# locuslab/mpc.pytorch

Measured on AMD Instinct MI355X. Metric: LQR problem-steps/sec (batch*T/s), n_state=12 n_ctrl=4 T=50, higher is better.
Workload: dtype f32

## Files before the change

### mpc.pytorch_amd/csrc/capi.hip

```cpp
#include <algorithm>
#include <atomic>
#include <cmath>
#include <cstdio>
#include <cstdlib>
#include <cstring>
#include <string>

#include "lqr_common.h"

namespace mpclqr {
static thread_local std::string g_last_error;
void set_last_error(const char *msg) { g_last_error = msg ? msg : ""; }

static int fail(int code, const char *msg)
{
    set_last_error(msg);
    return code;
}

template <typename F>
static int by_dtype(int dtype, F &&f)
{
    return dtype == MPC_F32 ? f(float()) : f(double());
}

struct EnvSwitch { const char *name; char a, b; int unset; };
static const EnvSwitch SW_DPP16_RING = {"MPC_DPP16_RING", '2', '4', 0};
static const EnvSwitch SW_MFMA40_RING = {"MPC_MFMA40_RING", '2', '3', 0};
static const EnvSwitch SW_DPP16_RESIDENT = {"MPC_DPP16_RESIDENT", '0', '1', -1};
static int read_switch(const EnvSwitch &s)
{
    const char *e = getenv(s.name);
    return (e && (e[0] == s.a || e[0] == s.b)) ? e[0] - '0' : s.unset;
}

struct DeviceFacts {
    int ring_force;
    int simds;
    int ring40_force;
    bool sticky;
    int resident;
};
static const DeviceFacts &device_facts()
{
    static DeviceFacts f = [] {
        DeviceFacts d;
        d.simds = 1024;
        hipDeviceProp_t prop;
        int dev = 0;
        if (hipGetDevice(&dev) == hipSuccess && hipGetDeviceProperties(&prop, dev) == hipSuccess && prop.multiProcessorCount > 0)
            d.simds = prop.multiProcessorCount * 4;
        d.ring_force = read_switch(SW_DPP16_RING);
        d.ring40_force = read_switch(SW_MFMA40_RING);
        d.sticky = getenv("MPC_DPP16_RING_DYNAMIC") == nullptr;
        d.resident = read_switch(SW_DPP16_RESIDENT);
        return d;
    }();
    return f;
}
static int env_switch(const EnvSwitch &s, int at_load) { return device_facts().sticky ? at_load : read_switch(s); }

#ifndef MPC_DPP16_RESIDENT_DEFAULT
#define MPC_DPP16_RESIDENT_DEFAULT 1
#endif
static std::atomic<int64_t> g_resident_launches{0};
static bool dpp16_resident(const StepParams<float> &q)
{
    const DeviceFacts &f = device_facts();
    int on = env_switch(SW_DPP16_RESIDENT, f.resident);
    const int waves = (q.B + 3) / 4;
    if (on < 0) on = (MPC_DPP16_RESIDENT_DEFAULT && 16 * (long)waves > 15 * (long)f.simds) ? 1 : 0;
    return on != 0 && q.bound_mode == MPC_BOUND_NONE && !q.zero_mask && q.T >= 2 && q.T <= 64  && !q.sweep_only &&
           (q.B + 3) / 4 <= f.simds;
}

static int mfma40_ring(const StepParams<float> &sp)
{
    const DeviceFacts &f = device_facts();
    const int force = env_switch(SW_MFMA40_RING, f.ring40_force);
    if (force) return force;
    if (sp.bound_mode != MPC_BOUND_NONE) return sp.B > f.simds ? 2 : 3;
    return (sp.B > f.simds && sp.B <= f.simds + f.simds / 2) ? 2 : 3;
}

static int check_problem(const mpc_lqr_problem *p, bool need_cost, bool need_nominal, bool need_F = true)
{
    if (!p) return fail(MPC_E_NULL, "problem is NULL");
    if (p->B < 0 || p->T < 1 || p->ns < 1 || p->nc < 1) return fail(MPC_E_DIMS, "need B>=0, T>=1, ns>=1, nc>=1");
    if (p->nc > 64) return fail(MPC_E_DIMS, "n_ctrl > 64 is not supported");
    if (p->dtype != MPC_F32 && p->dtype != MPC_F64) return fail(MPC_E_DTYPE, "dtype must be MPC_F32 or MPC_F64");
    if (p->B == 0) return MPC_OK;
    if (need_cost && (!p->C || !p->c)) return fail(MPC_E_NULL, "C / c is NULL");
    if (need_F && p->T > 1 && !p->F) return fail(MPC_E_NULL, "F is NULL");
    if (!p->x_init) return fail(MPC_E_NULL, "x_init is NULL");
    if (need_nominal && (!p->cur_x || !p->cur_u)) return fail(MPC_E_NULL, "current_x / current_u is NULL");
    return MPC_OK;
}

static int check_env(const mpc_env_dynamics *e, int ns, int nc)
{
    const int kind = e->kind & ~MPC_ENV_CTRL_CARRY, carry = (e->kind & MPC_ENV_CTRL_CARRY) ? 1 : 0;
    if (kind < MPC_ENV_PENDULUM || kind > MPC_ENV_CARTPOLE) return fail(MPC_E_ARG, "unknown simulator kind");
    if (!e->params) return fail(MPC_E_NULL, "simulator params is NULL");
    if (nc != 1 || ns != env_ns(kind) + carry) return fail(MPC_E_DIMS, "n_state / n_ctrl do not match the simulator");
    if (!(e->dt > 0) || !(e->u_max >= 0)) return fail(MPC_E_ARG, "simulator dt / u_max");
    return MPC_OK;
}

static int check_env_points(const mpc_env_dynamics *env, int dtype, int64_t N)
{
    if (!env) return fail(MPC_E_NULL, "simulator is NULL");
    if (dtype != MPC_F32 && dtype != MPC_F64) return fail(MPC_E_DTYPE, "bad dtype");
    if (env->kind & MPC_ENV_CTRL_CARRY) return fail(MPC_E_UNSUPPORTED, "MPC_ENV_CTRL_CARRY: linearise the simulator itself (the carry block is constant)");
    if (env->kind < MPC_ENV_PENDULUM || env->kind > MPC_ENV_CARTPOLE) return fail(MPC_E_ARG, "unknown simulator kind");
    const int rc = check_env(env, env_ns(env->kind), 1);
    if (rc) return rc;
    return N < 0 ? fail(MPC_E_DIMS, "N < 0") : MPC_OK;
}

static int check_options(const mpc_lqr_problem *p, const mpc_lqr_options *o)
{
    if (!o) return MPC_OK;
    if (o->bound_mode < MPC_BOUND_NONE || o->bound_mode > MPC_BOUND_TENSOR) return fail(MPC_E_ARG, "bad bound_mode");
    if (o->bound_mode == MPC_BOUND_TENSOR && (!o->lo || !o->hi) && p->B > 0) return fail(MPC_E_NULL, "tensor bounds are NULL");
    if (o->max_linesearch_iter < 1) return fail(MPC_E_ARG, "max_linesearch_iter must be > 0");
    if (o->delta_u == o->delta_u && o->delta_u >= 0 && o->bound_mode == MPC_BOUND_NONE)
        return fail(MPC_E_ARG, "delta_u requires u_lower/u_upper (mpc/lqr_step.py:195)");
    if (o->true_dynamics) {
        int rc = check_env(o->true_dynamics, p->ns, p->nc);
        if (rc) return rc;
    }
    return MPC_OK;
}


static mpc_lqr_problem sizes_only(int B, int T, int ns, int nc, int dtype)
{
    mpc_lqr_problem q;
    memset(&q, 0, sizeof(q));
    q.B = B; q.T = T; q.ns = ns; q.nc = nc; q.dtype = dtype;
    return q;
}
template <typename real>
static StepParams<real> sizes_only(const StepParams<real> &sp)
{
    const mpc_lqr_problem q = sizes_only(sp.B, sp.T, sp.ns, sp.nc, sizeof(real) == 4 ? MPC_F32 : MPC_F64);
    StepParams<real> s = make_params<real>(&q, nullptr, nullptr);
    s.env.kind = sp.env.kind;
    return s;
}

struct WsLayout { int64_t K, k, Kk, bytes, qp, qp_st, qp_sb; };
static WsLayout layout_generic(int64_t TB, int B, int ns, int nc, int64_t e) { return {0, TB * nc * ns * e, -1, TB * nc * (ns + 1) * e, -1, 0, 0}; }
static WsLayout layout_row(int64_t TB, int B, int ns, int nc, int64_t e) { return {0, TB * nc * ns * e, 0, TB * nc * (ns + 1) * e * 9, -1, 0, 0}; }
static WsLayout layout_fused12(int64_t TB, int B, int ns, int nc, int64_t e) { return {0, TB * nc * ns * e, 0, e == 4 ? TB * (128 + 16) * 4 : TB * 64 * 8, -1, 0, 0}; }
static WsLayout layout_dpp16(int64_t TB, int B, int ns, int nc, int64_t e) { return {0, TB * nc * ns * e, 0, layout_fused12(TB, B, ns, nc, e).bytes, 48 * 4, (int64_t)B * 64, 64}; }
static WsLayout layout_mfma40(int64_t TB, int B, int ns, int nc, int64_t e)
{
    const WsLayout w = layout_generic(TB, B, ns, nc, e);
    return {w.K, w.k, w.bytes, w.bytes + TB * (328 + 40) * 4, w.k, (int64_t)B * nc, nc};
}
static WsLayout layout_pad40(int64_t TB, int B, int ns, int nc, int64_t e)
{
    const int64_t k = TB * 256 * 4, Kk = k + TB * 8 * 4;
    return {0, k, Kk, Kk + TB * (328 + 40) * 4, k, (int64_t)B * 8, 8};
}

static bool row_kernel_pays(long lds_bytes, int B)
{
    const long per_cu = (160L * 1024) / lds_bytes;
    return (B + 3) / 4 <= (device_facts().simds / 4) * (per_cu < 8 ? per_cu : 8);
}
static bool wave1_pays(const StepParams<float> &sp) { return wave1_supported(sp) && row_kernel_pays(wave1_lds_bytes(sp), sp.B); }
static bool wave1_pays(const StepParams<double> &) { return false; }
static bool wave1_carry_pays(const StepParams<float> &sp) { return wave1_carry_supported(sp) && row_kernel_pays(wave1_carry_lds_bytes(sp), sp.B); }

static int dpp16_ring(const StepParams<float> &sp)
{
    const bool constrained = sp.bound_mode != MPC_BOUND_NONE || sp.zero_mask != nullptr;
    const int force = env_switch(SW_DPP16_RING, device_facts().ring_force);
    return (force ? force == 2 : (!constrained || (sp.B + 3) / 4 > device_facts().simds)) ? 2 : 4;
}
static int launch_dpp16(const StepRoute &r, const StepParams<float> &q, hipStream_t st)
{
    if (r.ring == 2 && dpp16_resident(q)) {
        g_resident_launches.fetch_add(1, std::memory_order_relaxed);
        return launch_step_dpp16_res(q, st);
    }
    return r.ring == 2 ? launch_step_dpp16_ring2(q, st) : launch_step_dpp16(q, st);
}

enum StepFamily { FAM_NONE, FAM_GENERIC, FAM_ROW , FAM_FUSED12 ,
                  FAM_MFMA40 , FAM_PAD40  };
enum {
    K_SIMULATOR = 1,
    K_CARRIES = 2,
    K_CARRY_ONLY = 4,
    K_SWEEP_STOP = 8,
    K_PARKS_STATUS = 16,
    K_SIZES_QUERY = 32,
    K_SIZES_RECORD = 64,
};
struct StepRefusal { int code; const char *text; };
template <typename real>
struct StepKernelIn {
    bool (*rule)(const StepParams<real> &);
    int (*launch)(const StepRoute &, const StepParams<real> &, hipStream_t);
    bool needs_workspace;
// ... 772 lines not shown
                       const void *gf, void *gparams, void *workspace, int64_t workspace_bytes, void *stream)
{
    const int rc = check_env_points(env, dtype, N);
    if (rc || N == 0) return rc;
    if (!x || !u || !gF || !gf || !gparams || !workspace) return fail(MPC_E_NULL, "env_param_grad: NULL argument");
    if (workspace_bytes < env_param_grad_workspace_bytes(N))
        return fail(MPC_E_DIMS, "workspace too small (see mpc_env_param_grad_workspace_bytes)");
    if ((uintptr_t)workspace % 8) return fail(MPC_E_ARG, "env_param_grad: the workspace must be 8-byte aligned");
    return by_dtype(dtype, [&](auto t) {
        typedef decltype(t) real;
        EnvDesc<real> e;
        set_env(e, env);
        return launch_env_param_grad<real>(e, (long)N, (const real *)x, (const real *)u, (const real *)gF, (const real *)gf, (real *)gparams,
                                           (double *)workspace, (hipStream_t)stream);
    });
}

int64_t mpc_mlp_workspace_bytes(const mpc_mlp_dynamics *net) { return nn_workspace_bytes(net); }

int mpc_mlp_supported(const mpc_mlp_dynamics *net, int n_state, int n_ctrl) { return nn_budget(net, n_state, n_ctrl); }

int mpc_mlp_rollout(const mpc_lqr_problem *p, const mpc_lqr_options *o, const mpc_mlp_dynamics *net, const void *K,
                    const void *k, const void *old_costs, const mpc_lqr_outputs *out, void *workspace,
                    int64_t workspace_bytes, void *stream)
{
    if (!p || !out) return fail(MPC_E_NULL, "problem / outputs is NULL");
    if (p->B < 0 || p->T < 1 || p->ns < 1 || p->nc < 1) return fail(MPC_E_DIMS, "need B>=0, T>=1, ns>=1, nc>=1");
    if (p->dtype != MPC_F32) return fail(MPC_E_DTYPE, "the network kernels are fp32 only");
    if (p->B == 0) return MPC_OK;
    if (!p->x_init || !p->cur_u) return fail(MPC_E_NULL, "x_init / current_u is NULL");
    if ((p->C == nullptr) != (p->c == nullptr)) return fail(MPC_E_NULL, "pass both C and c, or neither");
    if (!out->new_x) return fail(MPC_E_NULL, "new_x is NULL");
    if ((K == nullptr) != (k == nullptr)) return fail(MPC_E_NULL, both_gains);
    if (K) {
        if (!p->cur_x || !p->C || !old_costs || !out->new_u)
            return fail(MPC_E_NULL, "line search needs current_x, C, c, old_costs and new_u");
        int rc = check_options(p, o);
        if (rc) return rc;
        if (o && o->true_dynamics) return fail(MPC_E_ARG, "mpc_mlp_rollout: options.true_dynamics must be NULL");
    }
    StepParams<float> sp = make_params<float>(p, K ? o : nullptr, out);
    sp.K = (float *)K;
    sp.k = (float *)k;
    sp.old_costs_in = (const float *)old_costs;
    return launch_nn_rollout(sp, net, workspace, workspace_bytes, (hipStream_t)stream);
}

int mpc_mlp_linearize(const mpc_mlp_dynamics *net, int n_state, int n_ctrl, int64_t N, const void *x, const void *u,
                      void *F, void *f, void *workspace, int64_t workspace_bytes, void *stream)
{
    if (n_state < 1 || n_ctrl < 1 || N < 0) return fail(MPC_E_DIMS, "need n_state>=1, n_ctrl>=1, N>=0");
    if (N == 0) return MPC_OK;
    if (!x || !u || !F || !f) return fail(MPC_E_NULL, "mlp_linearize: NULL argument");
    return launch_nn_linearize(net, (long)N, n_state, n_ctrl, (const float *)x, (const float *)u, (float *)F, (float *)f,
                               workspace, workspace_bytes, (hipStream_t)stream);
}

int mpc_mlp_linearize_carry(const mpc_mlp_dynamics *net, int n_state, int n_ctrl, int64_t N, const void *z, const void *u,
                            void *aF, void *af, void *workspace, int64_t workspace_bytes, void *stream)
{
    if (n_state < 1 || n_ctrl < 1 || N < 0) return fail(MPC_E_DIMS, "need n_state>=1, n_ctrl>=1, N>=0");
    if (n_state + n_ctrl > 32) return fail(MPC_E_DIMS, "mlp_linearize_carry: n_state + n_ctrl <= 32 (the augmented state of the step kernels)");
    if (N == 0) return MPC_OK;
    if (!z || !u || !aF || !af) return fail(MPC_E_NULL, "mlp_linearize_carry: NULL argument");
    return launch_nn_linearize_carry(net, (long)N, n_state, n_ctrl, (const float *)z, (const float *)u, (float *)aF, (float *)af,
                                     workspace, workspace_bytes, (hipStream_t)stream);
}

int64_t mpc_mlp_param_grad_workspace_bytes(const mpc_mlp_dynamics *net, int64_t N) { return nn_param_grad_workspace_bytes(net, N); }

int mpc_mlp_param_grad(const mpc_mlp_dynamics *net, int n_state, int n_ctrl, int64_t N, const void *x, const void *u,
                       const void *gF, const void *gf, const mpc_mlp_param_grads *out, void *workspace,
                       int64_t workspace_bytes, void *stream)
{
    if (n_state < 1 || n_ctrl < 1 || N < 0) return fail(MPC_E_DIMS, "need n_state>=1, n_ctrl>=1, N>=0");
    if (!net || !out || !workspace) return fail(MPC_E_NULL, "mlp_param_grad: NULL argument");
    if (N > 0 && (!x || !u || !gF || !gf)) return fail(MPC_E_NULL, "mlp_param_grad: NULL argument");
    if (net->n_layers >= 1 && net->n_layers <= MPC_MLP_MAX_LAYERS)
        for (int l = 0; l < net->n_layers; ++l)
            if (!out->gW[l] || !out->gb[l]) return fail(MPC_E_NULL, "mlp_param_grad: gradient pointer is NULL");
    return launch_nn_param_grad(net, (long)N, n_state, n_ctrl, (const float *)x, (const float *)u, (const float *)gF,
                                (const float *)gf, out, workspace, workspace_bytes, (hipStream_t)stream);
}

int mpc_lqr_kkt_prepare(int dtype, int B, int T, int ns, int nc, const void *dl_dx, const void *dl_du,
                        const void *u_star, const mpc_lqr_options *o, void *negr, uint8_t *mask, void *stream)
{
    if (dtype != MPC_F32 && dtype != MPC_F64) return fail(MPC_E_DTYPE, "bad dtype");
    if (B < 0 || T < 1 || ns < 1 || nc < 1) return fail(MPC_E_DIMS, "bad dims");
    if (B == 0) return MPC_OK;
    if (!dl_dx || !dl_du || !negr) return fail(MPC_E_NULL, "kkt_prepare: NULL argument");
    const int mode = o ? o->bound_mode : MPC_BOUND_NONE;
    if (mask && (mode == MPC_BOUND_NONE || !u_star)) return fail(MPC_E_ARG, "kkt_prepare: mask needs bounds and u*");
    if (mask && mode == MPC_BOUND_TENSOR && (!o->lo || !o->hi)) return fail(MPC_E_NULL, "tensor bounds are NULL");
    return by_dtype(dtype, [&](auto t) {
        typedef decltype(t) real;
        return launch_kkt_prepare<real>(B, T, ns, nc, (const real *)dl_dx, (const real *)dl_du, (const real *)u_star, mode, o ? (real)o->lo_s : 0,
                                        o ? (real)o->hi_s : 0, o ? (const real *)o->lo : nullptr, o ? (const real *)o->hi : nullptr, (real *)negr,
                                        mask, (hipStream_t)stream);
    });
}

int mpc_pnqp_lu(int dtype, int B, int n, const void *H, const void *q, const void *lo, const void *hi,
                const void *x0, int n_iter, void *x, uint8_t *If_out, int32_t *iters, int32_t *status,
                void *Hfree, void *LU, int32_t *pivots, void *stream)
{
    if (dtype != MPC_F32 && dtype != MPC_F64) return fail(MPC_E_DTYPE, "bad dtype");
    if (B < 0 || n < 1) return fail(MPC_E_DIMS, "bad dims");
    if (B == 0) return MPC_OK;
    if (!H || !q || !lo || !hi || !x) return fail(MPC_E_NULL, "pnqp: NULL argument");
    if (n_iter < 1) n_iter = 20;
    return by_dtype(dtype, [&](auto t) {
        typedef decltype(t) real;
        return launch_pnqp<real>(B, n, (const real *)H, (const real *)q, (const real *)lo, (const real *)hi, (const real *)x0, n_iter, (real *)x,
                                 If_out, iters, status, (real *)Hfree, (real *)LU, pivots, (hipStream_t)stream);
    });
}

int mpc_pnqp(int dtype, int B, int n, const void *H, const void *q, const void *lo, const void *hi,
             const void *x0, int n_iter, void *x, uint8_t *If_out, int32_t *iters, int32_t *status,
             void *Hfree, void *stream)
{
    return mpc_pnqp_lu(dtype, B, n, H, q, lo, hi, x0, n_iter, x, If_out, iters, status, Hfree, nullptr, nullptr, stream);
}

int mpc_traj_cost(const mpc_lqr_problem *p, void *x, void *cost, void *stream)
{
    if (!p) return fail(MPC_E_NULL, "problem is NULL");
    int rc = check_problem(p, cost != nullptr, false);
    if (rc) return rc;
    if (p->B == 0) return MPC_OK;
    if (!p->cur_u) return fail(MPC_E_NULL, "traj_cost: u (cur_u) is NULL");
    hipStream_t st = (hipStream_t)stream;
    if (p->dtype == MPC_F32) {
        StepParams<float> sp = make_params<float>(p, nullptr, nullptr);
        if (!cost && x && traj_wave_supported(sp)) return launch_traj_wave(sp, (float *)x, st);
        return launch_traj_cost<float>(sp, (float *)x, (float *)cost, st);
    }
    StepParams<double> sp = make_params<double>(p, nullptr, nullptr);
    return launch_traj_cost<double>(sp, (double *)x, (double *)cost, st);
}

int mpc_select_best(int dtype, int B, int T, int ns, int nc, int first, double best_cost_eps, const void *x,
                    const void *u, const void *costs, const void *du_norm, void *best_x, void *best_u,
                    void *best_costs, void *best_du_norm, void *flags, void *host_flags, int32_t host_tag,
                    const int32_t *status, void *stream)
{
    if (dtype != MPC_F32 && dtype != MPC_F64) return fail(MPC_E_DTYPE, "bad dtype");
    if (B < 0 || T < 1 || ns < 1 || nc < 1) return fail(MPC_E_DIMS, "bad dims");
    if (B == 0) return MPC_OK;
    if (!x || !u || !costs || !du_norm || !best_x || !best_u || !best_costs || !best_du_norm || !flags)
        return fail(MPC_E_NULL, "select_best: NULL argument");
    if ((uintptr_t)flags & 7 || (uintptr_t)host_flags & 7) return fail(MPC_E_ARG, "select_best: the flags blocks must be 8-byte aligned");
    return by_dtype(dtype, [&](auto t) {
        typedef decltype(t) real;
        return launch_select_best<real>(B, T, ns, nc, first, (real)best_cost_eps, (const real *)x, (const real *)u, (const real *)costs,
                                        (const real *)du_norm, (real *)best_x, (real *)best_u, (real *)best_costs, (real *)best_du_norm, flags,
                                        host_flags, host_tag, status, (hipStream_t)stream);
    });
}

int mpc_du_norm_reference(int dtype, int T, int B, int nc, const void *u, const void *new_u, void *out, void *stream)
{
    if (dtype != MPC_F32 && dtype != MPC_F64) return fail(MPC_E_DTYPE, "bad dtype");
    if (B < 0 || T < 1 || nc < 1) return fail(MPC_E_DIMS, "bad dims");
    if (B == 0) return MPC_OK;
    if (!u || !new_u || !out) return fail(MPC_E_NULL, "du_norm_reference: NULL argument");
    hipStream_t st = (hipStream_t)stream;
    if (dtype == MPC_F32) return launch_du_norm_reference<float>(T, B, nc, (const float *)u, (const float *)new_u, (float *)out, st);
    return launch_du_norm_reference<double>(T, B, nc, (const double *)u, (const double *)new_u, (double *)out, st);
}

}
```

### mpc.pytorch_amd/csrc/lqr_common.h

```cpp
#pragma once
#include <hip/hip_runtime.h>
#include <stdint.h>
#include "../../include/mpc_lqr.h"
#include "lqr_params.h"

namespace mpclqr {

void set_last_error(const char *msg);

enum { MPC_IMPL_AUTO = 0, MPC_IMPL_GENERIC = 1, MPC_IMPL_MFMA16 = 2, MPC_IMPL_DPP16 = 3, MPC_IMPL_TINY = 4, MPC_IMPL_MFMA40 = 5,
       MPC_IMPL_WAVE1 = 6, MPC_IMPL_MFMA40_PAD = 7, MPC_IMPL_DPP16_PAD = 8,
       MPC_IMPL_MFMA40_NARROW = 9,
       MPC_IMPL_WAVE1_CARRY = 10 };

struct StepRoute {
    int code; const char *msg;
    int kernel;
    int phase;
    int ring;
    bool pad16;
    bool needs_resolve;
    int64_t K_off, k_off;
    int64_t Kk_off, status_off;
    int64_t qp_off, qp_st, qp_sb;
};
template <typename real>
StepRoute step_route(const StepParams<real> &sp, const mpc_lqr_problem *p, int impl, int phase_mask, const void *workspace,
                     int64_t workspace_bytes);

struct KktPointers {
    const void *dl_dx, *dl_du, *dC, *dc, *dF, *df, *dx_init, *dx_out, *du_out, *workspace;
};
struct KktRoute {
    int code; const char *msg;
    bool no_kernel;
    int kernel;
    int64_t bytes;
};
KktRoute kkt_fused_route(const StepParams<float> &sp, const mpc_lqr_problem *p, const KktPointers &a, int64_t workspace_bytes);
KktRoute kkt_fused_route_kernel(const StepParams<float> &sp, const mpc_lqr_problem *p, const KktPointers &a, int64_t workspace_bytes,
                                int kernel);

template <typename real> int launch_step_generic(const StepParams<real> &p, int phase_mask, hipStream_t st);
template <typename real> int launch_pnqp(int B, int n, const real *H, const real *q, const real *lo,
                                         const real *hi, const real *x0, int n_iter, real *x,
                                         uint8_t *If_out, int *iters, int *status, real *Hfree,
                                         real *LU, int *pivots, hipStream_t st);
template <typename real> int launch_traj_cost(const StepParams<real> &p, real *x, real *cost, hipStream_t st);
template <typename real> int launch_kkt_grads(const StepParams<real> &p, const real *dx, const real *du,
                                              const real *dl_dx, const real *dl_du, real *dC, real *dc,
                                              real *dF, real *df, real *dx_init, hipStream_t st);
template <typename real> int launch_kkt_prepare(int B, int T, int ns, int nc, const real *dl_dx,
                                                const real *dl_du, const real *u_star, int bound_mode,
                                                real lo_s, real hi_s, const real *lo, const real *hi,
                                                real *negr, uint8_t *mask, hipStream_t st);
template <typename real> int launch_select_best(int B, int T, int ns, int nc, int first, real eps,
                                                const real *x, const real *u, const real *costs,
                                                const real *du_norm, real *bx, real *bu, real *bc,
                                                real *bd, void *flags, void *host_flags, int host_tag, const int *status,
                                                hipStream_t st);
template <typename real> int launch_du_norm_reference(int T, int B, int nc, const real *u, const real *new_u, real *out, hipStream_t st);
template <typename real> int launch_env_linearize(const EnvDesc<real> &env, long N, const real *x, const real *u,
                                                  real *F, real *f, hipStream_t st);
int64_t env_param_grad_workspace_bytes(int64_t N);
template <typename real> int launch_env_param_grad(const EnvDesc<real> &env, long N, const real *x, const real *u,
                                                   const real *gF, const real *gf, real *gparams, double *ws, hipStream_t st);
size_t generic_lds_bytes(int ns, int nc, size_t elem);
template <typename real> int launch_slew_augment(const mpc_lqr_problem *p, double gamma, real *aC, real *ac, real *aF, real *af, hipStream_t st);

bool dpp16_supported(const StepParams<float> &p);
int launch_step_dpp16(const StepParams<float> &p, hipStream_t st);
int launch_step_dpp16_ring2(const StepParams<float> &p, hipStream_t st);
bool dpp16_pad_supported(const StepParams<float> &p);
int launch_step_dpp16_res(const StepParams<float> &p, hipStream_t st);
int launch_step_dpp16_pad(const StepParams<float> &p, hipStream_t st);
bool kkt_dpp16_supported(const StepParams<float> &p, const float *dx, const float *du, const float *dl_dx,
                         const float *dC, const float *dF);
int launch_kkt_dpp16(const StepParams<float> &p, const float *dx, const float *du, const float *dl_dx, float *dC,
                     float *dc, float *dF, float *df, float *dx_init, hipStream_t st);

bool kkt_fused_dpp16_supported(const StepParams<float> &p, const float *dl_dx, const float *dl_du, const float *dC,
                               const float *dF, const float *ws);
int64_t kkt_fused_dpp16_workspace_bytes(int T, int B);
bool kkt_fused_dpp16_pad_supported(const StepParams<float> &p, const float *ws);
int launch_kkt_fused_dpp16_pad(const StepParams<float> &p, const float *dl_dx, const float *dl_du, float *dC, float *dc, float *dF,
                               float *df, float *dx_init, float *dx_out, float *du_out, float *ws, float decay, int max_ls,
                               hipStream_t st);
int launch_kkt_fused_dpp16(const StepParams<float> &p, const float *dl_dx, const float *dl_du, float *dC, float *dc, float *dF,
                           float *df, float *dx_init, float *dx_out, float *du_out, float *ws, float decay, int max_ls,
                           hipStream_t st);

bool tiny_supported(int ns, int nc);
template <typename real> int launch_step_tiny(const StepParams<real> &p, hipStream_t st);
bool wave1_supported(const StepParams<float> &p);
long wave1_lds_bytes(const StepParams<float> &p);
int launch_step_wave1(const StepParams<float> &p, hipStream_t st);
bool wave1_carry_supported(const StepParams<float> &p);
long wave1_carry_lds_bytes(const StepParams<float> &p);
int launch_step_wave1_carry(const StepParams<float> &p, hipStream_t st);

bool traj_wave_supported(const StepParams<float> &p);
int launch_traj_wave(const StepParams<float> &p, float *x, hipStream_t st);
bool kkt_wave_supported(const StepParams<float> &p, const float *dx, const float *du, const float *dl_dx, const float *dC,
                        const float *dF);
int launch_kkt_wave(const StepParams<float> &p, const float *dx, const float *du, const float *dl_dx, float *dC,
                    float *dc, float *dF, float *df, float *dx_init, hipStream_t st);

int launch_kkt_costates(const StepParams<float> &p, const float *dx, const float *du, const float *dl_dx, float *park, float *dx_init,
                        hipStream_t st);
int kkt_shared_partials(int T, int B);
int64_t kkt_shared_workspace_bytes(int T, int B, int ns, int nc);
int launch_kkt_shared(const StepParams<float> &p, const float *dx, const float *du, const float *dl_dx, float *sum_dC, float *sum_dc,
                      float *sum_dF, float *sum_df, float *dx_init, void *workspace, hipStream_t st);

int launch_kkt_outer(const StepParams<float> &p, const float *dx, const float *du, float *dC, float *dc, float *dF, hipStream_t st);

bool mfma40_supported(const StepParams<float> &p);
int launch_step_mfma40(const StepParams<float> &p, hipStream_t st);
int launch_step_mfma40_ring2(const StepParams<float> &p, hipStream_t st);
bool mfma40_pad_supported(const StepParams<float> &p);
bool mfma40_pad16_supported(const StepParams<float> &p);
int launch_step_mfma40_pad4(const StepParams<float> &p, hipStream_t st);
int launch_step_mfma40_pad16(const StepParams<float> &p, hipStream_t st);
bool mfma40_narrow_supported(const StepParams<float> &p);
int launch_step_mfma40_narrow4(const StepParams<float> &p, hipStream_t st);
int launch_step_mfma40_narrow16(const StepParams<float> &p, hipStream_t st);
bool kkt_fused_mfma40_supported(const StepParams<float> &p, const float *dl_dx, const float *dl_du, const float *dC,
                                const float *dF, const float *ws);
int64_t kkt_fused_mfma40_workspace_bytes(int T, int B);
bool kkt_fused_mfma40_pad_supported(const StepParams<float> &p, const float *ws);
bool kkt_fused_mfma40_pad16_supported(const StepParams<float> &p, const float *ws);
int launch_kkt_fused_mfma40_pad16(const StepParams<float> &p, const float *dl_dx, const float *dl_du, float *dC, float *dc, float *dF,
                                  float *df, float *dx_init, float *dx_out, float *du_out, float *ws, float decay, int max_ls,
                                  hipStream_t st);
int launch_kkt_fused_mfma40_pad(const StepParams<float> &p, const float *dl_dx, const float *dl_du, float *dC, float *dc, float *dF,
                                float *df, float *dx_init, float *dx_out, float *du_out, float *ws, float decay, int max_ls,
                                hipStream_t st);
int launch_kkt_fused_mfma40(const StepParams<float> &p, const float *dl_dx, const float *dl_du, float *dC, float *dc, float *dF,
                            float *df, float *dx_init, float *dx_out, float *du_out, float *ws, float decay, int max_ls,
                            hipStream_t st);
bool kkt_fused_mfma40_narrow_supported(const StepParams<float> &p, const float *ws);
bool kkt_fused_mfma40_narrow16_supported(const StepParams<float> &p, const float *ws);
int64_t kkt_fused_mfma40_narrow_workspace_bytes(int T, int B);
int launch_kkt_fused_mfma40_narrow16(const StepParams<float> &p, const float *dl_dx, const float *dl_du, float *dC, float *dc, float *dF,
                                     float *df, float *dx_init, float *dx_out, float *du_out, float *ws, float decay, int max_ls,
                                     hipStream_t st);
int launch_kkt_fused_mfma40_narrow4(const StepParams<float> &p, const float *dl_dx, const float *dl_du, float *dC, float *dc, float *dF,
                                    float *df, float *dx_init, float *dx_out, float *du_out, float *ws, float decay, int max_ls,
                                    hipStream_t st);

int nn_budget(const mpc_mlp_dynamics *net, int ns, int nc);
int64_t nn_workspace_bytes(const mpc_mlp_dynamics *net);
int launch_nn_rollout(const StepParams<float> &p, const mpc_mlp_dynamics *net, void *workspace, int64_t bytes, hipStream_t st);
int launch_nn_linearize(const mpc_mlp_dynamics *net, long N, int ns, int nc, const float *x, const float *u, float *F,
                        float *f, void *workspace, int64_t bytes, hipStream_t st);
int launch_nn_linearize_carry(const mpc_mlp_dynamics *net, long N, int ns, int nc, const float *z, const float *u, float *aF,
                              float *af, void *workspace, int64_t bytes, hipStream_t st);
int64_t nn_param_grad_workspace_bytes(const mpc_mlp_dynamics *net, int64_t N);
int launch_nn_param_grad(const mpc_mlp_dynamics *net, long N, int ns, int nc, const float *x, const float *u, const float *gF,
                         const float *gf, const mpc_mlp_param_grads *out, void *workspace, int64_t bytes, hipStream_t st);

bool mfma16_supported(const StepParams<float> &p);
int launch_step_mfma16(const StepParams<float> &p, hipStream_t st);
bool mfma16_supported(const StepParams<double> &p);
int launch_step_mfma16(const StepParams<double> &p, hipStream_t st);

}
```

### mpc.pytorch_amd/csrc/lqr_generic.hip

```cpp
#include "lqr_common.h"

namespace mpclqr {

namespace {

constexpr int WAVE = 64;
constexpr int MAX_THREADS = 256;

inline int threads_for(int ns, int nc) { return (ns + nc) > 24 ? MAX_THREADS : WAVE; }

template <typename real> __device__ __forceinline__ real rabs(real x) { return x < 0 ? -x : x; }
template <typename real> __device__ __forceinline__ real rsqrt_(real x);
template <> __device__ __forceinline__ float rsqrt_<float>(float x) { return sqrtf(x); }
template <> __device__ __forceinline__ double rsqrt_<double>(double x) { return sqrt(x); }

template <typename real> __device__ __forceinline__ real eclamp(real x, real lo, real hi)
{
    if (x < lo) x = lo;
    if (x > hi) x = hi;
    return x;
}

typedef float mfma_acc_t __attribute__((ext_vector_type(4)));
template <class LA, class LB>
// ... 699 lines not shown
    const int ir = i < ns ? i : 0;
    const bool hasf = p.f != nullptr;
    const bool isu = i >= ns && i < n;
    const real *aux0 = isu ? p.cur_u + (long)b * nc + (i - ns) : (hasf && i < ns ? p.f + (long)b * p.f_sb + i : p.x_init);
    const long aux_st = isu ? (long)B * nc : (hasf && i < ns ? p.f_st : 0);
    const bool auxv = isu || (hasf && i < ns);
    const real *F0 = p.F + (long)b * p.F_sb + (long)ir * n;
    auto load_stage = [&](int t, int slot) {
        t = t < T - 2 ? t : T - 2;
        const real *Ft = F0 + (long)t * p.F_st;
        if constexpr (VEC) {
            const float4 *F4 = reinterpret_cast<const float4 *>(Ft);
#pragma unroll
            for (int q = 0; q < 4; ++q) {
                const float4 v = F4[q];
                row[slot][4 * q] = v.x, row[slot][4 * q + 1] = v.y, row[slot][4 * q + 2] = v.z, row[slot][4 * q + 3] = v.w;
            }
        } else {
#pragma unroll
            for (int j = 0; j < 16; ++j) row[slot][j] = Ft[j < n ? j : 0];
        }
        aux[slot] = aux0[(long)t * aux_st];
    };
    auto advance = [&](int t, int slot) {
        const real a = auxv ? aux[slot] : (real)0;
        const real tau = i < ns ? xi : a;
        real acc = i < ns ? a : (real)0;
#pragma unroll
        for (int j = 0; j < 16; ++j) acc += (VEC || j < n ? row[slot][j] : (real)0) * __shfl(tau, j, 16);
        xi = acc;
        if (own) x[((long)(t + 1) * B + b) * ns + i] = xi;
    };
#pragma unroll
    for (int d = 0; d < DEPTH; ++d) load_stage(d, d);
    int t0 = 0;
    for (; t0 + DEPTH <= T - 1; t0 += DEPTH) {
#pragma unroll
        for (int d = 0; d < DEPTH; ++d) {
            advance(t0 + d, d);
            load_stage(t0 + d + DEPTH, d);
        }
    }
#pragma unroll
    for (int d = 0; d < DEPTH - 1; ++d)
        if (t0 + d < T - 1) advance(t0 + d, d);
}

template <typename real>
__global__ void __launch_bounds__(MAX_THREADS)
kkt_grads_kernel(StepParams<real> p, const real *dx, const real *du, const real *dl_dx, const real *dl_du,
                 real *dC, real *dc, real *dF, real *df, real *dx_init)
{
    extern __shared__ __attribute__((aligned(16))) char smem_raw[];
    Smem<real> s;
    s.carve(smem_raw, p.ns, p.nc, blockDim.x);
    const int b = blockIdx.x, tid = threadIdx.x, nt = blockDim.x;
    const int ns = p.ns, nc = p.nc, n = ns + nc, T = p.T, B = p.B;
    if (b >= B) return;
    real *lam = s.xn, *dlam = s.dxv, *lam2 = s.xn2, *dlam2 = s.v;
    bool have = false;
    for (int t = T - 1; t >= 0; --t) {
        const long tb = (long)t * B + b;
        const real *Ct = p.C + (long)t * p.C_st + (long)b * p.C_sb;
        const real *ct = p.c + (long)t * p.c_st + (long)b * p.c_sb;
        for (int e = tid; e < n * n; e += nt) s.Q[e] = Ct[e];
        if (have) {
            const real *Ft = p.F + (long)t * p.F_st + (long)b * p.F_sb;
            for (int e = tid; e < ns * n; e += nt) s.F[e] = Ft[e];
        }
        for (int i = tid; i < n; i += nt) {
            s.tau[i] = i < ns ? p.cur_x[tb * ns + i] : p.cur_u[tb * nc + (i - ns)];
            s.dtau[i] = i < ns ? dx[tb * ns + i] : du[tb * nc + (i - ns)];
        }
        __syncthreads();
        for (int e = tid; e < n * n; e += nt) {
            const int i = e / n, j = e - i * n;
            dC[tb * n * n + e] = (real)-0.5 * (s.dtau[i] * s.tau[j] + s.tau[i] * s.dtau[j]);
        }
        for (int i = tid; i < n; i += nt) dc[tb * n + i] = -s.dtau[i];
        for (int i = tid; i < ns; i += nt) {
            real r1 = 0, r2 = 0;
            for (int j = 0; j < n; ++j) {
                r1 += s.Q[i * n + j] * s.tau[j];
                r2 += s.Q[i * n + j] * s.dtau[j];
            }
            r1 += ct[i];
            r2 -= dl_dx[tb * ns + i];
            if (have)
                for (int m = 0; m < ns; ++m) {
                    r1 += s.F[m * n + i] * lam[m];
                    r2 += s.F[m * n + i] * dlam[m];
                }
            lam2[i] = r1;
            dlam2[i] = r2;
        }
        if (have) {
            for (int e = tid; e < ns * n; e += nt) {
                const int i = e / n, j = e - i * n;
                dF[tb * ns * n + e] = -(dlam[i] * s.tau[j] + lam[i] * s.dtau[j]);
            }
            if (df)
                for (int i = tid; i < ns; i += nt) df[tb * ns + i] = -dlam[i];
        }
        __syncthreads();
        for (int i = tid; i < ns; i += nt) { lam[i] = lam2[i]; dlam[i] = dlam2[i]; }
        __syncthreads();
        have = true;
    }
    for (int i = tid; i < ns; i += nt) dx_init[(long)b * ns + i] = -dlam[i];
}

template <typename real>
__global__ void kkt_prepare_kernel(long TB, int ns, int nc, const real *dl_dx, const real *dl_du,
                                   const real *u_star, int bound_mode, real lo_s, real hi_s,
                                   const real *lo, const real *hi, real *negr, uint8_t *mask)
{
    const int n = ns + nc;
    const long total = TB * n;
    for (long e = (long)blockIdx.x * blockDim.x + threadIdx.x; e < total; e += (long)gridDim.x * blockDim.x) {
        const long tb = e / n;
        const int i = (int)(e - tb * n);
        if (i < ns) {
            negr[e] = -dl_dx[tb * ns + i];
        } else {
            const long ui = tb * nc + (i - ns);
            negr[e] = -dl_du[ui];
            if (mask) {
                const real l = bound_mode == MPC_BOUND_SCALAR ? lo_s : lo[ui];
                const real h = bound_mode == MPC_BOUND_SCALAR ? hi_s : hi[ui];
                const real u = u_star[ui];
                mask[ui] = (rabs<real>(u - l) <= (real)1e-8 || rabs<real>(u - h) <= (real)1e-8) ? 1 : 0;
            }
        }
    }
}

template <typename real> struct BitsOf;
template <> struct BitsOf<float> { using type = unsigned int; };
template <> struct BitsOf<double> { using type = unsigned long long; };

constexpr int kSelPB = 8;

template <typename real> struct SelectArgs {
    int B, T, ns, nc, first;
    real eps;
    const real *x, *u, *costs, *du;
    real *bx, *bu, *bc, *bd;
    const int *status;
    unsigned char *flags, *host;
    int host_tag;
};

template <typename real, typename vec>
__global__ void __launch_bounds__(256) select_best_kernel(SelectArgs<real> a, int owners_only)
{
    constexpr int VW = sizeof(vec) / sizeof(real);
    const int tid = threadIdx.x;
    if (blockIdx.x == 0 && !owners_only) {
        __shared__ real s_max[4];
        __shared__ int s_fl[4];
        const volatile real *bc = a.bc;
        real d = 0;
        int fl = 0;
        for (int b = tid; b < a.B; b += 256) {
            real v = a.du[b];
            if (a.first || a.costs[b] <= bc[b] + a.eps) fl |= 1;
            if (v != v) { fl |= 2; v = 0; }
            d = v > d ? v : d;
            if (a.status && (a.status[b] & (MPC_ST_C_ASYMMETRIC | MPC_ST_C_TESTED)) != MPC_ST_C_TESTED) fl |= 4;
        }
        for (int off = 32; off > 0; off >>= 1) {
            const real o = __shfl_down(d, off);
            d = o > d ? o : d;
            fl |= __shfl_down(fl, off);
        }
        if ((tid & 63) == 0) s_max[tid >> 6] = d, s_fl[tid >> 6] = fl;
        __syncthreads();
        if (tid == 0) {
            for (int w = 1; w < 4; ++w) d = s_max[w] > d ? s_max[w] : d, fl |= s_fl[w];
            if (fl & 2) d = (real)NAN;
            const int word = (((fl & 1) && !a.first) ? 1 : 0) | ((fl & 4) ? 2 : 0);
            *reinterpret_cast<int *>(a.flags) = word;
            *reinterpret_cast<real *>(a.flags + 8) = d;
            if (a.host) {
                *reinterpret_cast<volatile int *>(a.host) = word;
                *reinterpret_cast<volatile real *>(a.host + 8) = d;
                __threadfence_system();
                *reinterpret_cast<volatile int *>(a.host + 4) = a.host_tag;
                __threadfence_system();
            }
        }
        return;
    }
    __shared__ int s_take[kSelPB];
    const int b0 = (blockIdx.x - (owners_only ? 0 : 1)) * kSelPB;
    const int nb = a.B - b0 < kSelPB ? a.B - b0 : kSelPB;
    if (tid < nb) {
        const int b = b0 + tid;
        const real cnew = a.costs[b];
        const int take = a.first || cnew <= a.bc[b] + a.eps;
        if (take) {
            a.bc[b] = cnew;
            a.bd[b] = a.du[b];
        }
        s_take[tid] = take;
    }
    __syncthreads();
    const int wx = nb * a.ns / VW, wu = nb * a.nc / VW, W = wx + wu;
    const vec *__restrict__ x = reinterpret_cast<const vec *>(a.x), *__restrict__ u = reinterpret_cast<const vec *>(a.u);
    vec *__restrict__ bx = reinterpret_cast<vec *>(a.bx), *__restrict__ bu = reinterpret_cast<vec *>(a.bu);
    const int total = a.T * W;
    for (int it = tid; it < total; it += 256) {
        const int t = it / W, r = it - t * W;
        const bool isx = r < wx;
        const int e = isx ? r : r - wx, d = isx ? a.ns : a.nc;
        if (!s_take[e * VW / d]) continue;
        const long at = ((long)t * a.B + b0) * d / VW + e;
        if (isx) bx[at] = x[at];
        else bu[at] = u[at];
    }
}

inline int check_launch(const char *what)
{
    hipError_t e = hipGetLastError();
    if (e != hipSuccess) {
        set_last_error((std::string(what) + ": " + hipGetErrorString(e)).c_str());
        return MPC_E_LAUNCH;
    }
    return MPC_OK;
}

}

size_t generic_lds_bytes(int ns, int nc, size_t elem)
{
    const size_t n = (size_t)ns + nc;
    size_t cnt = n * n + ns * n + n * ns + (size_t)ns * ns + (size_t)nc * (nc + 1 + ns) + (size_t)nc * ns +
                 (size_t)nc * (ns + 1) + n + ns + n + n + (size_t)nc * 8 + (size_t)ns * 3 + MAX_THREADS;
    return cnt * elem + (size_t)nc * sizeof(int) + 16;
}

template <typename real> int launch_step_generic(const StepParams<real> &p, int phase_mask, hipStream_t st)
{
    const size_t lds = generic_lds_bytes(p.ns, p.nc, sizeof(real));
    if (lds > 160 * 1024) { set_last_error("n_state/n_ctrl too large for the LDS-resident generic kernel"); return MPC_E_DIMS; }
    if (lds > 64 * 1024)
        (void)hipFuncSetAttribute(reinterpret_cast<const void *>(&lqr_step_generic_kernel<real>),
                                  hipFuncAttributeMaxDynamicSharedMemorySize, (int)lds);
    const int grid = p.gate ? (p.B < 1024 ? p.B : 1024) : p.B;
    hipLaunchKernelGGL(lqr_step_generic_kernel<real>, dim3(grid), dim3(threads_for(p.ns, p.nc)), lds, st, p, phase_mask);
    return check_launch("lqr_step_generic_kernel");
}

template <typename real>
int launch_pnqp(int B, int n, const real *H, const real *q, const real *lo, const real *hi, const real *x0,
                int n_iter, real *x, uint8_t *If_out, int *iters, int *status, real *Hfree, real *LU, int *pivots,
                hipStream_t st)
{
    const size_t lds = ((size_t)n * (n + 1) + 7 * (size_t)n) * sizeof(real) + 2 * (size_t)n * sizeof(int) + 16;
    if (lds > 160 * 1024) { set_last_error("pnqp: n too large for LDS"); return MPC_E_DIMS; }
    if (lds > 64 * 1024)
        (void)hipFuncSetAttribute(reinterpret_cast<const void *>(&pnqp_kernel<real>),
                                  hipFuncAttributeMaxDynamicSharedMemorySize, (int)lds);
    const int threads = n <= 32 ? 64 : (n <= 64 ? 128 : 256);
    hipLaunchKernelGGL(pnqp_kernel<real>, dim3(B), dim3(threads), lds, st, B, n, H, q, lo, hi, x0, n_iter, x,
                       If_out, iters, status, Hfree, LU, pivots);
    return check_launch("pnqp_kernel");
}

template <typename real>
__global__ void __launch_bounds__(64) env_traj_lane_kernel(StepParams<real> p, real *x)
{
    const int b = blockIdx.x * 64 + threadIdx.x;
    if (b >= p.B) return;
    const int ns = p.ns, T = p.T, B = p.B;
    real xi[6], xn[6];
    for (int i = 0; i < ns; ++i) {
        xi[i] = p.x_init[(long)b * ns + i];
        x[(long)b * ns + i] = xi[i];
    }
    real u = T > 1 ? p.cur_u[b] : (real)0;
    for (int t = 0; t < T - 1; ++t) {
        const real un = t + 1 < T - 1 ? p.cur_u[(long)(t + 1) * B + b] : (real)0;
        if (!p.env.carry) env_step<real>(p.env, xi, u, xn, nullptr);
        else if (p.env.kind == MPC_ENV_CARTPOLE) env_step_carry<real, 5>(p.env, xi, u, xn, nullptr);
        else env_step_carry<real, 3>(p.env, xi, u, xn, nullptr);
        for (int i = 0; i < ns; ++i) {
            xi[i] = xn[i];
            x[((long)(t + 1) * B + b) * ns + i] = xn[i];
        }
        u = un;
    }
}

template <typename real> int launch_traj_cost(const StepParams<real> &p, real *x, real *cost, hipStream_t st)
{
    if (!cost && x && p.env.kind && p.nc == 1 && p.ns <= 6) {
        hipLaunchKernelGGL(env_traj_lane_kernel<real>, dim3((unsigned)((p.B + 63) / 64)), dim3(64), 0, st, p, x);
        return check_launch("env_traj_lane_kernel");
    }
    if (!cost && x && !p.env.kind && p.ns + p.nc <= 16) {
        const long groups = p.B;
        const dim3 grid((unsigned)((groups * 16 + 255) / 256));
        bool vec = false;
        if constexpr (sizeof(real) == 4)
            vec = p.ns + p.nc == 16 && ((uintptr_t)p.F & 15) == 0 && p.F_st % 4 == 0 && p.F_sb % 4 == 0;
        if (vec) hipLaunchKernelGGL((traj_rows16_kernel<real, sizeof(real) == 4>), grid, dim3(256), 0, st, p, x);
        else hipLaunchKernelGGL((traj_rows16_kernel<real, false>), grid, dim3(256), 0, st, p, x);
        return check_launch("traj_rows16_kernel");
    }
    const size_t lds = generic_lds_bytes(p.ns, p.nc, sizeof(real));
    if (lds > 160 * 1024) { set_last_error("traj_cost: dims too large"); return MPC_E_DIMS; }
    if (lds > 64 * 1024)
        (void)hipFuncSetAttribute(reinterpret_cast<const void *>(&traj_cost_kernel<real>),
                                  hipFuncAttributeMaxDynamicSharedMemorySize, (int)lds);
    hipLaunchKernelGGL(traj_cost_kernel<real>, dim3(p.B), dim3(threads_for(p.ns, p.nc)), lds, st, p, x, cost);
    return check_launch("traj_cost_kernel");
}

template <typename real>
int launch_kkt_grads(const StepParams<real> &p, const real *dx, const real *du, const real *dl_dx,
                     const real *dl_du, real *dC, real *dc, real *dF, real *df, real *dx_init, hipStream_t st)
{
    const size_t lds = generic_lds_bytes(p.ns, p.nc, sizeof(real));
    if (lds > 160 * 1024) { set_last_error("kkt_grads: dims too large"); return MPC_E_DIMS; }
    if (lds > 64 * 1024)
        (void)hipFuncSetAttribute(reinterpret_cast<const void *>(&kkt_grads_kernel<real>),
                                  hipFuncAttributeMaxDynamicSharedMemorySize, (int)lds);
    hipLaunchKernelGGL(kkt_grads_kernel<real>, dim3(p.B), dim3(threads_for(p.ns, p.nc)), lds, st, p, dx, du, dl_dx, dl_du, dC, dc,
                       dF, df, dx_init);
    return check_launch("kkt_grads_kernel");
}

template <typename real>
int launch_kkt_prepare(int B, int T, int ns, int nc, const real *dl_dx, const real *dl_du, const real *u_star,
                       int bound_mode, real lo_s, real hi_s, const real *lo, const real *hi, real *negr,
                       uint8_t *mask, hipStream_t st)
{
    const long TB = (long)T * B;
    const long total = TB * (ns + nc);
    int blocks = (int)((total + 255) / 256);
    if (blocks > 4096) blocks = 4096;
    if (blocks < 1) blocks = 1;
    hipLaunchKernelGGL(kkt_prepare_kernel<real>, dim3(blocks), dim3(256), 0, st, TB, ns, nc, dl_dx, dl_du, u_star,
                       bound_mode, lo_s, hi_s, lo, hi, negr, mask);
    return check_launch("kkt_prepare_kernel");
}

template <typename real>
int launch_select_best(int B, int T, int ns, int nc, int first, real eps, const real *x, const real *u,
                       const real *costs, const real *du_norm, real *bx, real *bu, real *bc, real *bd,
                       void *flags, void *host_flags, int host_tag, const int *status, hipStream_t st)
{
    SelectArgs<real> a{B, T, ns, nc, first, eps, x, u, costs, du_norm, bx, bu, bc, bd, status,
                       (unsigned char *)flags, (unsigned char *)host_flags, host_tag};
    const unsigned owners = (unsigned)((B + kSelPB - 1) / kSelPB);
    bool vec4 = false;
    if constexpr (sizeof(real) == 4)
        vec4 = ns % 4 == 0 && nc % 4 == 0 && (((uintptr_t)x | (uintptr_t)bx | (uintptr_t)u | (uintptr_t)bu) & 15) == 0;
    auto go = [&](unsigned grid, int owners_only) {
        if (vec4) hipLaunchKernelGGL((select_best_kernel<real, float4>), dim3(grid), dim3(256), 0, st, a, owners_only);
        else hipLaunchKernelGGL((select_best_kernel<real, real>), dim3(grid), dim3(256), 0, st, a, owners_only);
    };
    if (eps >= 0) go(1 + owners, 0);
    else {
        go(1, 0);
        go(owners, 1);
    }
    return check_launch("select_best_kernel");
}

template <typename real>
__global__ void __launch_bounds__(256) du_norm_reference_kernel(int T, int B, int nc, const real *u, const real *new_u, real *out)
{
    const long row = (long)T * nc;
    const long f0 = (long)blockIdx.x * row;
    real acc = 0;
    for (long i = threadIdx.x; i < row; i += blockDim.x) {
        const long f = f0 + i;
        const long b = f % B, ta = f / B;
        const long src = (ta / nc * B + b) * nc + ta % nc;
        const real d = u[src] - new_u[src];
        acc += d * d;
    }
    __shared__ real part[256];
    part[threadIdx.x] = acc;
    __syncthreads();
    for (int s = 128; s > 0; s >>= 1) {
        if ((int)threadIdx.x < s) part[threadIdx.x] += part[threadIdx.x + s];
        __syncthreads();
    }
    if (threadIdx.x == 0) out[blockIdx.x] = rsqrt_<real>(part[0]);
}

template <typename real>
int launch_du_norm_reference(int T, int B, int nc, const real *u, const real *new_u, real *out, hipStream_t st)
{
    hipLaunchKernelGGL(du_norm_reference_kernel<real>, dim3(B), dim3(256), 0, st, T, B, nc, u, new_u, out);
    return check_launch("du_norm_reference_kernel");
}

template <typename real>
__global__ void env_linearize_kernel(EnvDesc<real> env, long N, const real *x, const real *u, real *F, real *f)
{
    const long i = (long)blockIdx.x * blockDim.x + threadIdx.x;
    if (i >= N) return;
    const int ns = env_ns(env.kind), n = ns + 1;
    real xi[5], out[5], J[30];
    for (int j = 0; j < ns; ++j) xi[j] = x[i * ns + j];
    const real ui = u[i];
    env_step<real>(env, xi, ui, out, J);
    for (int r = 0; r < ns; ++r) {
        real acc = out[r];
        for (int j = 0; j < ns; ++j) acc -= J[r * n + j] * xi[j];
        acc -= J[r * n + ns] * ui;
        f[i * ns + r] = acc;
        for (int j = 0; j < n; ++j) F[(i * ns + r) * n + j] = J[r * n + j];
    }
}

template <typename real>
int launch_env_linearize(const EnvDesc<real> &env, long N, const real *x, const real *u, real *F, real *f,
                         hipStream_t st)
{
    if (N <= 0) return MPC_OK;
    hipLaunchKernelGGL(env_linearize_kernel<real>, dim3((unsigned)((N + 255) / 256)), dim3(256), 0, st, env, N, x,
                       u, F, f);
    return check_launch("env_linearize_kernel");
}

#define INSTANTIATE(real)                                                                                     \
    template int launch_step_generic<real>(const StepParams<real> &, int, hipStream_t);                        \
    template int launch_pnqp<real>(int, int, const real *, const real *, const real *, const real *,          \
                                   const real *, int, real *, uint8_t *, int *, int *, real *, real *, int *, \
                                   hipStream_t);                                                              \
    template int launch_traj_cost<real>(const StepParams<real> &, real *, real *, hipStream_t);                \
    template int launch_kkt_grads<real>(const StepParams<real> &, const real *, const real *, const real *,   \
                                        const real *, real *, real *, real *, real *, real *, hipStream_t);   \
    template int launch_kkt_prepare<real>(int, int, int, int, const real *, const real *, const real *, int,   \
                                          real, real, const real *, const real *, real *, uint8_t *,          \
                                          hipStream_t);                                                       \
    template int launch_env_linearize<real>(const EnvDesc<real> &, long, const real *, const real *, real *,   \
                                            real *, hipStream_t);                                             \
    template int launch_du_norm_reference<real>(int, int, int, const real *, const real *, real *, hipStream_t); \
    template int launch_select_best<real>(int, int, int, int, int, real, const real *, const real *,          \
                                          const real *, const real *, real *, real *, real *, real *, void *, \
                                          void *, int, const int *, hipStream_t);
INSTANTIATE(float)
INSTANTIATE(double)

}
```

Measured before the change: 2.281 billion.

## Rewrite select_best with vectorized batched flag scan and strided owner copy

Replaces the select_best kernel with a new version. Block 0 scans du_norm, costs, best costs and status with 16-byte vector and nontemporal loads in large per-thread batches, then reduces the flag word and max du with wave shuffles. Owner blocks copy the chosen trajectories using a layout that maps threads over (time, element) with several loads in flight. The old kernel stays available behind MPC_SELECT_SERIAL. It adds code complexity, and select_best may be a small part of the LQR throughput metric.

New measurement: 2.280 billion, median of 4. About the same (-0.0%).

```diff
diff --git a/mpc.pytorch_amd/csrc/capi.hip b/mpc.pytorch_amd/csrc/capi.hip
--- a/mpc.pytorch_amd/csrc/capi.hip
+++ b/mpc.pytorch_amd/csrc/capi.hip
@@ -28,6 +28,7 @@
 static const EnvSwitch SW_DPP16_RING = {"MPC_DPP16_RING", '2', '4', 0};
 static const EnvSwitch SW_MFMA40_RING = {"MPC_MFMA40_RING", '2', '3', 0};
 static const EnvSwitch SW_DPP16_RESIDENT = {"MPC_DPP16_RESIDENT", '0', '1', -1};
+static const EnvSwitch SW_SELECT_SERIAL = {"MPC_SELECT_SERIAL", '0', '1', 0};
 static int read_switch(const EnvSwitch &s)
 {
     const char *e = getenv(s.name);
@@ -40,6 +41,7 @@
     int ring40_force;
     bool sticky;
     int resident;
+    int select_serial;
 };
 static const DeviceFacts &device_facts()
 {
@@ -54,6 +56,7 @@
         d.ring40_force = read_switch(SW_MFMA40_RING);
         d.sticky = getenv("MPC_DPP16_RING_DYNAMIC") == nullptr;
         d.resident = read_switch(SW_DPP16_RESIDENT);
+        d.select_serial = read_switch(SW_SELECT_SERIAL);
         return d;
     }();
     return f;
@@ -1132,11 +1135,12 @@
     if (!x || !u || !costs || !du_norm || !best_x || !best_u || !best_costs || !best_du_norm || !flags)
         return fail(MPC_E_NULL, "select_best: NULL argument");
     if ((uintptr_t)flags & 7 || (uintptr_t)host_flags & 7) return fail(MPC_E_ARG, "select_best: the flags blocks must be 8-byte aligned");
+    const int serial = env_switch(SW_SELECT_SERIAL, device_facts().select_serial);
     return by_dtype(dtype, [&](auto t) {
         typedef decltype(t) real;
         return launch_select_best<real>(B, T, ns, nc, first, (real)best_cost_eps, (const real *)x, (const real *)u, (const real *)costs,
                                         (const real *)du_norm, (real *)best_x, (real *)best_u, (real *)best_costs, (real *)best_du_norm, flags,
-                                        host_flags, host_tag, status, (hipStream_t)stream);
+                                        host_flags, host_tag, status, serial, (hipStream_t)stream);
     });
 }
 
diff --git a/mpc.pytorch_amd/csrc/lqr_common.h b/mpc.pytorch_amd/csrc/lqr_common.h
--- a/mpc.pytorch_amd/csrc/lqr_common.h
+++ b/mpc.pytorch_amd/csrc/lqr_common.h
@@ -58,7 +58,7 @@
                                                 const real *x, const real *u, const real *costs,
                                                 const real *du_norm, real *bx, real *bu, real *bc,
                                                 real *bd, void *flags, void *host_flags, int host_tag, const int *status,
-                                                hipStream_t st);
+                                                int serial, hipStream_t st);
 template <typename real> int launch_du_norm_reference(int T, int B, int nc, const real *u, const real *new_u, real *out, hipStream_t st);
 template <typename real> int launch_env_linearize(const EnvDesc<real> &env, long N, const real *x, const real *u,
                                                   real *F, real *f, hipStream_t st);
diff --git a/mpc.pytorch_amd/csrc/lqr_generic.hip b/mpc.pytorch_amd/csrc/lqr_generic.hip
--- a/mpc.pytorch_amd/csrc/lqr_generic.hip
+++ b/mpc.pytorch_amd/csrc/lqr_generic.hip
@@ -875,7 +875,7 @@
 };
 
 template <typename real, typename vec>
-__global__ void __launch_bounds__(256) select_best_kernel(SelectArgs<real> a, int owners_only)
+__global__ void __launch_bounds__(256) select_best_serial_kernel(SelectArgs<real> a, int owners_only)
 {
     constexpr int VW = sizeof(vec) / sizeof(real);
     const int tid = threadIdx.x;
@@ -944,6 +944,176 @@
     }
 }
 
+template <typename T> struct SelPack;
+template <> struct SelPack<float> { typedef float type __attribute__((ext_vector_type(4))); };
+template <> struct SelPack<double> { typedef double type __attribute__((ext_vector_type(2))); };
+template <> struct SelPack<int> { typedef int type __attribute__((ext_vector_type(4))); };
+
+template <bool NT, typename T> __device__ __forceinline__ void sel_load4(const T *p, T *v)
+{
+    typedef typename SelPack<T>::type P;
+    constexpr int N = 16 / sizeof(T);
+    const P *q = reinterpret_cast<const P *>(p);
+#pragma unroll
+    for (int i = 0; i < 4 / N; ++i) {
+        const P w = NT ? __builtin_nontemporal_load(q + i) : q[i];
+#pragma unroll
+        for (int j = 0; j < N; ++j) v[i * N + j] = w[j];
+    }
+}
+template <bool NT, typename T> __device__ __forceinline__ T sel_load1(const T *p) { return NT ? __builtin_nontemporal_load(p) : *p; }
+
+constexpr int kSelWordsPT = 16;
+constexpr int kSelWordsBatch = 256 * kSelWordsPT;
+
+template <typename real, bool WITH_ST> struct SelWords {
+    real d;
+    int fl;
+    __device__ __forceinline__ void add(const SelectArgs<real> &a, bool in_range, real v, real cnew, real bold, int st)
+    {
+        int f = (a.first || cnew <= bold + a.eps) ? 1 : 0;
+        if (v != v) { f |= 2; v = 0; }
+        if (WITH_ST && (st & (MPC_ST_C_ASYMMETRIC | MPC_ST_C_TESTED)) != MPC_ST_C_TESTED) f |= 4;
+        fl |= in_range ? f : 0;
+        d = (in_range && v > d) ? v : d;
+    }
+};
+
+template <typename real, bool WITH_ST>
+__device__ __forceinline__ void select_words_scan(const SelectArgs<real> &a, real &d_out, int &fl_out)
+{
+    const int tid = threadIdx.x, B = a.B;
+    const bool al = (((uintptr_t)a.du | (uintptr_t)a.costs | (uintptr_t)a.bc | (WITH_ST ? (uintptr_t)a.status : (uintptr_t)0)) & 15) == 0;
+    const int nvec = al ? B & ~3 : 0;
+    SelWords<real, WITH_ST> w{(real)0, 0};
+    const int tb = nvec + tid, tbc = tb < B ? tb : B - 1;
+    const real t_du = a.du[tbc], t_cn = a.costs[tbc], t_bo = sel_load1<true>(a.bc + tbc);
+    const int t_st = WITH_ST ? a.status[tbc] : 0;
+    for (int base = 0; base < nvec; base += kSelWordsBatch) {
+        real du[kSelWordsPT], cn[kSelWordsPT], bo[kSelWordsPT];
+        int st[kSelWordsPT];
+#pragma unroll
+        for (int k = 0; k < kSelWordsPT / 4; ++k) {
+            const int b = base + 4 * (k * 256 + tid), bcl = b < nvec ? b : nvec - 4;
+            sel_load4<false>(a.du + bcl, du + 4 * k);
+            sel_load4<false>(a.costs + bcl, cn + 4 * k);
+            sel_load4<true>(a.bc + bcl, bo + 4 * k);
+            if (WITH_ST) sel_load4<false>(a.status + bcl, st + 4 * k);
+        }
+#pragma unroll
+        for (int k = 0; k < kSelWordsPT; ++k)
+            w.add(a, base + 4 * ((k / 4) * 256 + tid) < nvec, du[k], cn[k], bo[k], WITH_ST ? st[k] : 0);
+    }
+    for (int base = nvec + 256; base < B; base += kSelWordsBatch) {
+        real du[kSelWordsPT], cn[kSelWordsPT], bo[kSelWordsPT];
+        int st[kSelWordsPT];
+#pragma unroll
+        for (int k = 0; k < kSelWordsPT; ++k) {
+            const int b = base + k * 256 + tid, bcl = b < B ? b : B - 1;
+            du[k] = a.du[bcl];
+            cn[k] = a.costs[bcl];
+            bo[k] = sel_load1<true>(a.bc + bcl);
+            st[k] = WITH_ST ? a.status[bcl] : 0;
+        }
+#pragma unroll
+        for (int k = 0; k < kSelWordsPT; ++k) w.add(a, base + k * 256 + tid < B, du[k], cn[k], bo[k], st[k]);
+    }
+    w.add(a, tb < B, t_du, t_cn, t_bo, t_st);
+    d_out = w.d;
+    fl_out = w.fl;
+}
+
+template <typename real> __device__ __forceinline__ void select_words(const SelectArgs<real> &a)
+{
+    __shared__ real s_max[4];
+    __shared__ int s_fl[4];
+    const int tid = threadIdx.x;
+    real d;
+    int fl;
+    if (a.status) select_words_scan<real, true>(a, d, fl);
+    else select_words_scan<real, false>(a, d, fl);
+    for (int off = 32; off > 0; off >>= 1) {
+        const real o = __shfl_down(d, off);
+        d = o > d ? o : d;
+        fl |= __shfl_down(fl, off);
+    }
+    if ((tid & 63) == 0) s_max[tid >> 6] = d, s_fl[tid >> 6] = fl;
+    __syncthreads();
+    if (tid == 0) {
+        for (int w = 1; w < 4; ++w) d = s_max[w] > d ? s_max[w] : d, fl |= s_fl[w];
+        if (fl & 2) d = (real)NAN;
+        const int word = (((fl & 1) && !a.first) ? 1 : 0) | ((fl & 4) ? 2 : 0);
+        *reinterpret_cast<int *>(a.flags) = word;
+        *reinterpret_cast<real *>(a.flags + 8) = d;
+        if (a.host) {
+            *reinterpret_cast<volatile int *>(a.host) = word;
+            *reinterpret_cast<volatile real *>(a.host + 8) = d;
+            __threadfence_system();
+            *reinterpret_cast<volatile int *>(a.host + 4) = a.host_tag;
+            __threadfence_system();
+        }
+    }
+}
+
+constexpr int kSelPieces = 8;
+template <typename real, int VW> struct SelPiece { typedef real type __attribute__((ext_vector_type(VW))); };
+template <typename real> struct SelPiece<real, 1> { typedef real type; };
+
+template <typename real, typename vec>
+__device__ __forceinline__ void select_owner(const SelectArgs<real> &a, int b0)
+{
+    constexpr int VW = sizeof(vec) / sizeof(real);
+    typedef typename SelPiece<real, VW>::type piece;
+    __shared__ int s_take[kSelPB];
+    const int tid = threadIdx.x;
+    const int nb = a.B - b0 < kSelPB ? a.B - b0 : kSelPB;
+    int take = 0;
+    if (tid < nb) {
+        const int b = b0 + tid;
+        const real cnew = a.costs[b], dnew = a.du[b], bold = a.bc[b];
+        take = a.first || cnew <= bold + a.eps;
+        if (take) {
+            a.bc[b] = cnew;
+            a.bd[b] = dnew;
+        }
+        s_take[tid] = take;
+    }
+    if (!__syncthreads_or(take)) return;
+    const int wx = nb * a.ns / VW, wu = nb * a.nc / VW, W = wx + wu;
+    int r = tid, rs = 256, t0 = 0, ts = 1;
+    if (W <= 256) {
+        ts = 256 / W;
+        t0 = tid / W;
+        r = t0 < ts ? tid - t0 * W : W;
+        rs = W;
+    }
+    const int np = (a.T - t0 + ts - 1) / ts;
+    for (; r < W; r += rs) {
+        const bool isx = r < wx;
+        const int e = isx ? r : r - wx, d = isx ? a.ns : a.nc;
+        if (!s_take[e * VW / d]) continue;
+        const long step = (long)a.B * d / VW * ts;
+        const long at = ((long)t0 * a.B + b0) * d / VW + e;
+        const piece *__restrict__ src = reinterpret_cast<const piece *>(isx ? a.x : a.u) + at;
+        piece *__restrict__ dst = reinterpret_cast<piece *>(isx ? a.bx : a.bu) + at;
+        for (int j = 0; j < np; j += kSelPieces) {
+            piece v[kSelPieces];
+#pragma unroll
+            for (int k = 0; k < kSelPieces; ++k) v[k] = src[(j + k < np ? j + k : np - 1) * step];
+#pragma unroll
+            for (int k = 0; k < kSelPieces; ++k)
+                if (j + k < np) dst[(j + k) * step] = v[k];
+        }
+    }
+}
+
+template <typename real, typename vec>
+__global__ void __launch_bounds__(256) select_best_kernel(SelectArgs<real> a, int owners_only)
+{
+    if (blockIdx.x == 0 && !owners_only) select_words<real>(a);
+    else select_owner<real, vec>(a, (int)(blockIdx.x - (owners_only ? 0 : 1)) * kSelPB);
+}
+
 inline int check_launch(const char *what)
 {
     hipError_t e = hipGetLastError();
@@ -1074,7 +1244,7 @@
 template <typename real>
 int launch_select_best(int B, int T, int ns, int nc, int first, real eps, const real *x, const real *u,
                        const real *costs, const real *du_norm, real *bx, real *bu, real *bc, real *bd,
-                       void *flags, void *host_flags, int host_tag, const int *status, hipStream_t st)
+                       void *flags, void *host_flags, int host_tag, const int *status, int serial, hipStream_t st)
 {
     SelectArgs<real> a{B, T, ns, nc, first, eps, x, u, costs, du_norm, bx, bu, bc, bd, status,
                        (unsigned char *)flags, (unsigned char *)host_flags, host_tag};
@@ -1083,7 +1253,10 @@
     if constexpr (sizeof(real) == 4)
         vec4 = ns % 4 == 0 && nc % 4 == 0 && (((uintptr_t)x | (uintptr_t)bx | (uintptr_t)u | (uintptr_t)bu) & 15) == 0;
     auto go = [&](unsigned grid, int owners_only) {
-        if (vec4) hipLaunchKernelGGL((select_best_kernel<real, float4>), dim3(grid), dim3(256), 0, st, a, owners_only);
+        if (serial) {
+            if (vec4) hipLaunchKernelGGL((select_best_serial_kernel<real, float4>), dim3(grid), dim3(256), 0, st, a, owners_only);
+            else hipLaunchKernelGGL((select_best_serial_kernel<real, real>), dim3(grid), dim3(256), 0, st, a, owners_only);
+        } else if (vec4) hipLaunchKernelGGL((select_best_kernel<real, float4>), dim3(grid), dim3(256), 0, st, a, owners_only);
         else hipLaunchKernelGGL((select_best_kernel<real, real>), dim3(grid), dim3(256), 0, st, a, owners_only);
     };
     if (eps >= 0) go(1 + owners, 0);
@@ -1169,7 +1342,7 @@
     template int launch_du_norm_reference<real>(int, int, int, const real *, const real *, real *, hipStream_t); \
     template int launch_select_best<real>(int, int, int, int, int, real, const real *, const real *,          \
                                           const real *, const real *, real *, real *, real *, real *, void *, \
-                                          void *, int, const int *, hipStream_t);
+                                          void *, int, const int *, int, hipStream_t);
 INSTANTIATE(float)
 INSTANTIATE(double)
 
```
